# langtech-bsc/quantool

Measured on AMD Instinct MI355X. Metric: quantized weights/sec (GPTQ int4, Llama-3-8B, 512 calib samples), higher is better.
Workload: dtype f32

## Files before the change

### quantool_amd/csrc/cholesky.hip

```cpp
#include <stdlib.h>
#include <string.h>

#include <map>
#include <tuple>
#include <vector>

#include "common.h"
#include "gemm3_tn.h"
#include "sgemm_tn.h"

namespace {

constexpr int NB = 128;
constexpr int NBO_MAX = 1024;
static int chol_block_env(const char* name) {
    const char* e = getenv(name);
    if (!e) return 0;
    int x = atoi(e) / 128 * 128;
    return x < 128 ? 128 : (x > NBO_MAX ? NBO_MAX : x);
}
struct G3Step {
    int n_items = 0, n_red = 0;
    size_t item_off = 0, red_off = 0;
};
// ... 316 lines not shown
#pragma unroll
        for (int a = 0; a < 4; ++a)
#pragma unroll
            for (int r = 0; r < 16; ++r) {
                const int row = 32 * a + (r & 3) + 8 * (r >> 2) + 4 * h;
                if (row < n) Z[(size_t)row * ldz + col] = acc[a][r];
            }
    }
}

__global__ __launch_bounds__(128) void trinv_batched_kernel(const float* __restrict__ Rd_all, int K,
                                                            float* __restrict__ Dinv_all,
                                                            float* __restrict__ Y, int64_t ldy, int64_t bsW, int64_t bsY) {
    if (blockIdx.y) {
        Rd_all += (size_t)blockIdx.y * bsW;
        Dinv_all += (size_t)blockIdx.y * bsW;
        Y += (size_t)blockIdx.y * bsY;
    }
    extern __shared__ __attribute__((aligned(16))) float sm[];
    float* Rt = sm;
    float* Xs = sm + NB * LDT;
    const int b = blockIdx.x;
    const int n = (K - b * NB < NB) ? K - b * NB : NB;
    const float* Rd = Rd_all + (size_t)b * RD_STRIDE;
    const int j = threadIdx.x;
    for (int e = j; e < NB * NB; e += NB) {
        const int i = e / NB, c = e % NB;
        Rt[c * LDT + i] = Rd[e];
    }
    __syncthreads();
    float x0[32], x1[32], x2[32], x3[32];
#pragma unroll
    for (int r = 0; r < 32; ++r) {
        x0[r] = (r == j) ? 1.0f : 0.0f;
        x1[r] = (32 + r == j) ? 1.0f : 0.0f;
        x2[r] = (64 + r == j) ? 1.0f : 0.0f;
        x3[r] = (96 + r == j) ? 1.0f : 0.0f;
    }
#pragma unroll 1
    for (int pb = 3; pb >= 0; --pb) {
#pragma unroll
        for (int pp = 31; pp >= 0; --pp) {
            const int p = 32 * pb + pp;
            const float* rp = Rt + p * LDT;
            const float xp = QT_SEL4(pb, x0[pp], x1[pp], x2[pp], x3[pp]) / rp[p];
            if (pb == 0) x0[pp] = xp;
            if (pb == 1) x1[pp] = xp;
            if (pb == 2) x2[pp] = xp;
            if (pb == 3) x3[pp] = xp;
#define QT_XUPD(arr, a, r_to)                                                 \
    _Pragma("unroll") for (int r4 = 0; r4 < (r_to); r4 += 4) {                 \
        const f32x4 v4 = *(const f32x4*)(rp + 32 * (a) + r4);                 \
        _Pragma("unroll") for (int e = 0; e < 4; ++e)                         \
            if (r4 + e < (r_to)) arr[r4 + e] = fmaf(-v4[e], xp, arr[r4 + e]); \
    }
            if (pb == 0) { QT_XUPD(x0, 0, pp) } else { QT_XUPD(x0, 0, 32) }
            if (pb == 1) { QT_XUPD(x1, 1, pp) } else if (pb > 1) { QT_XUPD(x1, 1, 32) }
            if (pb == 2) { QT_XUPD(x2, 2, pp) } else if (pb > 2) { QT_XUPD(x2, 2, 32) }
            if (pb == 3) { QT_XUPD(x3, 3, pp) }
#undef QT_XUPD
        }
    }
#pragma unroll
    for (int r = 0; r < 32; ++r) {
        Xs[r * LDP + j] = x0[r];
        Xs[(32 + r) * LDP + j] = x1[r];
        Xs[(64 + r) * LDP + j] = x2[r];
        Xs[(96 + r) * LDP + j] = x3[r];
    }
    __syncthreads();
    float* Dinv = Dinv_all + (size_t)b * NB * NB;
    float* Yd = Y + (size_t)(b * NB) * ldy + b * NB;
    for (int e = j; e < NB * NB; e += NB) {
        const int i = e / NB, jj = e % NB;
        const bool in = (i < n && jj < n);
        Dinv[e] = (in && jj >= i) ? Xs[i * LDP + jj] : 0.0f;
        if (in) Yd[(size_t)i * ldy + jj] = (jj <= i) ? Xs[jj * LDP + i] : 0.0f;
    }
}

__global__ __launch_bounds__(256) void trinv_mfma_kernel(const float* __restrict__ Rd_all, int K,
                                                         float* __restrict__ Dinv_all,
                                                         float* __restrict__ Y, int64_t ldy, int64_t bsW, int64_t bsY) {
    if (blockIdx.y) {
        Rd_all += (size_t)blockIdx.y * bsW;
        Dinv_all += (size_t)blockIdx.y * bsW;
        Y += (size_t)blockIdx.y * bsY;
    }
    extern __shared__ __attribute__((aligned(16))) float Rs[];
    const int blk = blockIdx.x;
    const int n = (K - blk * NB < NB) ? K - blk * NB : NB;
    const float* Rd = Rd_all + (size_t)blk * RD_STRIDE;
    const int tid = threadIdx.x, lane = tid & 63, wave = tid >> 6;
    {
        constexpr int NV = RD_STRIDE / 4 / 256;
        f32x4 v[NV];
#pragma unroll
        for (int r = 0; r < NV; ++r) v[r] = ((const f32x4*)Rd)[tid + 256 * r];
#pragma unroll
        for (int r = 0; r < NV; ++r) ((f32x4*)Rs)[tid + 256 * r] = v[r];
    }
    const float* D32 = Rs + NB * NB;
    const int l31 = lane & 31, h = lane >> 5;
    const int col = wave * 32 + l31;

    f32x16 acc[4];
#pragma unroll
    for (int a = 0; a < 4; ++a)
#pragma unroll
        for (int r = 0; r < 16; ++r) {
            const int row = 32 * a + (r & 3) + 8 * (r >> 2) + 4 * h;
            acc[a][r] = (row == col) ? 1.0f : 0.0f;
        }
    __syncthreads();

#pragma unroll
    for (int b = 0; b < 4; ++b) {
        f32x16 zb;
#pragma unroll
        for (int r = 0; r < 16; ++r) zb[r] = 0.0f;
#pragma unroll
        for (int r = 0; r < 16; ++r) {
            const int k = (r & 3) + 8 * (r >> 2) + 4 * h;
            const float av = D32[(b * 32 + k) * 32 + l31];
            zb = __builtin_amdgcn_mfma_f32_32x32x2f32(av, acc[b][r], zb, 0, 0, 0);
        }
        acc[b] = zb;
#pragma unroll
        for (int a = b + 1; a < 4; ++a) {
#pragma unroll
            for (int r = 0; r < 16; ++r) {
                const int k = (r & 3) + 8 * (r >> 2) + 4 * h;
                const float av = -Rs[(32 * b + k) * NB + 32 * a + l31];
                acc[a] = __builtin_amdgcn_mfma_f32_32x32x2f32(av, zb[r], acc[a], 0, 0, 0);
            }
        }
    }
    float* Dinv = Dinv_all + (size_t)blk * NB * NB;
    float* Yd = Y + (size_t)(blk * NB) * ldy + blk * NB;
#pragma unroll
    for (int a = 0; a < 4; ++a)
#pragma unroll
        for (int r = 0; r < 16; ++r) {
            const int row = 32 * a + (r & 3) + 8 * (r >> 2) + 4 * h;
            const bool in = row < n && col < n;
            const float z = (in && row >= col) ? acc[a][r] : 0.0f;
            Dinv[col * NB + row] = z;
            if (in) Yd[(size_t)row * ldy + col] = z;
        }
}

__global__ __launch_bounds__(256) void transpose_lower_block_kernel(const float* __restrict__ Y, int64_t ldy, int w,
                                                                    float* __restrict__ XT, int ldx, int64_t bsY,
                                                                    int64_t bsXT) {
    if (blockIdx.z) {
        Y += (size_t)blockIdx.z * bsY;
        XT += (size_t)blockIdx.z * bsXT;
    }
    __shared__ float tile[32][33];
    const int bx = blockIdx.x * 32, by = blockIdx.y * 32;
    const int tx = threadIdx.x & 31, ty = threadIdx.x >> 5;
    for (int r = ty; r < 32; r += 8) {
        const int m = bx + r, k = by + tx;
        tile[r][tx] = (m < w && k < w && k <= m) ? Y[(size_t)m * ldy + k] : 0.0f;
    }
    __syncthreads();
    for (int r = ty; r < 32; r += 8) {
        const int k = by + r, m = bx + tx;
        if (k < w && m < w) XT[(size_t)k * ldx + m] = tile[tx][r];
    }
}

__global__ __launch_bounds__(256) void flat_reverse_lower_to_upper_kernel(float* __restrict__ U, int K, int64_t bsU) {
    U += (size_t)blockIdx.z * bsU;
    const int j = blockIdx.x * blockDim.x + threadIdx.x;
    const int i = blockIdx.y;
    if (j >= K || j < i) return;
    const size_t e = (size_t)i * K + j;
    const size_t pe = (size_t)(K - 1 - i) * K + (K - 1 - j);
    if (i == j) {
        if (e <= pe) {
            const float t = U[e];
            U[e] = U[pe];
            U[pe] = t;
        }
    } else {
        U[e] = U[pe];
        U[pe] = 0.0f;
    }
}

__global__ __launch_bounds__(256) void identity_if_failed_kernel(float* __restrict__ U, int K,
                                                                 const int32_t* __restrict__ info, int64_t bsU) {
    if (info[blockIdx.z] == 0) return;
    U += (size_t)blockIdx.z * bsU;
    for (int i = blockIdx.x; i < K; i += gridDim.x)
        for (int j = threadIdx.x; j < K; j += blockDim.x) U[(size_t)i * K + j] = (i == j) ? 1.0f : 0.0f;
}

}

static size_t chol_problem_ws_bytes(int K, const CholG3Plan* g3) {
    const size_t nb = (K + NB - 1) / NB;
    const size_t split = (size_t)2048 * NB * NB * 4 + (size_t)NBO_MAX * K * 4;
    size_t n = (size_t)NB * K * 4 + (size_t)NBO_MAX * K * 4 + (size_t)NBO_MAX * NBO_MAX * 4 + nb * (NB * NB + RD_STRIDE) * 4 + split + 256;
    if (g3->any) n += 2 * qt_align_up((size_t)3 * K * K * 2, 256) + (size_t)g3->max_slabs * 256 * 256 * 4 + 256;
    return qt_align_up(n, 256);
}

extern "C" size_t qt_cholesky_inverse_upper_batched_workspace_bytes(int K, int n_problems) {
    if (K <= 0 || n_problems <= 0) return 0;
    int nbo_, nbi_;
    const CholG3Plan* g3 = chol_blocks(K, nbo_, nbi_);
    return (size_t)n_problems * chol_problem_ws_bytes(K, g3) + g3->blob_bytes + 512;
}

extern "C" size_t qt_cholesky_inverse_upper_workspace_bytes(int K) {
    return qt_cholesky_inverse_upper_batched_workspace_bytes(K, 1);
}

static int chol_run(float* A, int64_t strideA, int K, float* U, int64_t strideU, int32_t* info, int nprob, void* workspace,
                    size_t workspace_bytes, hipStream_t stream) {
    const size_t need = qt_cholesky_inverse_upper_batched_workspace_bytes(K, nprob);
    if (!workspace || workspace_bytes < need) {
        qt_set_error("qt_cholesky_inverse_upper: workspace %zu < required %zu", workspace_bytes, need);
        return QT_ERR_WORKSPACE;
    }
    const int nblk = (K + NB - 1) / NB;
    char* ws = (char*)qt_align_up((size_t)workspace, 256);
    int NBO, NBI;
    const CholG3Plan* g3 = chol_blocks(K, NBO, NBI);
    const size_t prob_bytes = chol_problem_ws_bytes(K, g3);
    const int64_t sW = (int64_t)(prob_bytes / 4);
    const int64_t sA = nprob > 1 ? strideA : 0, sU = nprob > 1 ? strideU : 0;
    float* T = (float*)ws;
    float* TI = T + (size_t)NB * K;
    float* XT = TI + (size_t)NBO_MAX * K;
    float* Rd = XT + (size_t)NBO_MAX * NBO_MAX;
    float* Dinv = Rd + (size_t)nblk * RD_STRIDE;
    float* split_ws = Dinv + (size_t)nblk * NB * NB;
    const size_t split_ws_bytes = (size_t)2048 * NB * NB * 4 + (size_t)NBO_MAX * K * 4;
    unsigned short *Rpl = nullptr, *Ypl = nullptr;
    float* g3_slabs = nullptr;
    char* g3_tab = nullptr;
    const int64_t plane_stride = (int64_t)K * K;
    if (g3->any) {
        char* q = (char*)qt_align_up((size_t)((char*)split_ws + split_ws_bytes), 256);
        Rpl = (unsigned short*)q;
        q += qt_align_up((size_t)3 * K * K * 2, 256);
        Ypl = (unsigned short*)q;
        q += qt_align_up((size_t)3 * K * K * 2, 256);
        g3_slabs = (float*)q;
        g3_tab = (char*)qt_align_up((size_t)(ws + (size_t)nprob * prob_bytes), 256);
        QT_HIP(hipMemcpyAsync(g3_tab, g3->blob, g3->blob_bytes, hipMemcpyHostToDevice, stream));
    }
    auto g3_row = [&](const G3Step& st, const unsigned short* Bplanes, int col_a0, int col_b0, int M, int N, float* C,
                      int64_t bsC, int mode) -> int {
        G3Args a;
        a.Apl = Rpl;
        a.Bpl = Bplanes;
        a.plane_stride = plane_stride;
        a.ld = K;
        a.rowA0 = a.rowB0 = 0;
        a.colA0 = col_a0;
        a.colB0 = col_b0;
        a.colmax = K;
        a.M = M;
        a.N = N;
        a.C = C;
        a.ldc = K;
        a.mode = mode;
        a.slabs = g3_slabs;
        a.items = (const G3Item*)(g3_tab + st.item_off);
        a.n_items = st.n_items;
        a.red = (const G3Red*)(g3_tab + st.red_off);
        a.n_red = st.n_red;
        a.batch = nprob;
        a.bsApl = a.bsBpl = sW * 2;
        a.bsC = bsC;
        a.bsSlabs = sW;
        return qt_gemm3_launch(a, stream);
    };
    auto sgemm = [&](SgemmArgs& g, int64_t bsA_, int64_t bsB_, int64_t bsC_) -> int {
        g.batch = nprob;
        g.bsA = bsA_;
        g.bsB = bsB_;
        g.bsCin = g.bsCout = bsC_;
        g.bs_split = sW;
        return qt_sgemm_tn(g, stream);
    };
    float* Y = U;
    const int64_t sY = sU;
    const size_t inv_lds = (size_t)(NB * LDT + NB * LDP) * sizeof(float);
    const size_t potf2_lds = (size_t)(NB * LDA + 4 * 32 * 32) * sizeof(float);
    static QtOncePerDevice lds_attr;
    QT_HIP(lds_attr.run([&] {
        hipError_t e = hipFuncSetAttribute((const void*)potf2_kernel, hipFuncAttributeMaxDynamicSharedMemorySize,
                                           (int)potf2_lds);
        if (e == hipSuccess)
            e = hipFuncSetAttribute((const void*)trsm_rt_kernel, hipFuncAttributeMaxDynamicSharedMemorySize,
                                    (int)(RD_STRIDE * sizeof(float)));
        if (e == hipSuccess)
            e = hipFuncSetAttribute((const void*)trinv_batched_kernel, hipFuncAttributeMaxDynamicSharedMemorySize,
                                    (int)inv_lds);
        if (e == hipSuccess)
            e = hipFuncSetAttribute((const void*)trinv_mfma_kernel, hipFuncAttributeMaxDynamicSharedMemorySize,
                                    (int)(RD_STRIDE * sizeof(float)));
        return e;
    }));
    QT_HIP(hipMemsetAsync(info, 0, sizeof(int32_t) * nprob, stream));
    const int prio = qt_chain_prio();

    for (int J0 = 0, Jb = 0; J0 < K; J0 += NBO, ++Jb) {
        const int J1 = (K - J0 < NBO) ? K : J0 + NBO;
        if (g3->any && J0 > 0) {
            const G3Step& st = g3->fac[Jb];
            float* C = A + (size_t)J0 * K + J0;
            if (st.n_items > 0) {
                int rc = g3_row(st, Rpl, J0, J0, J1 - J0, K - J0, C, sA, G3_SUB);
                if (rc) return rc;
            } else {
                SgemmArgs g;
                g.A = A + J0; g.lda = K;
                g.B = A + J0; g.ldb = K;
                g.Cin = C; g.ldcin = K;
                g.Cout = C; g.ldcout = K;
                g.M = J1 - J0; g.N = K - J0; g.kdim = J0; g.k_mode = SG_K_FULL; g.mode = SG_MODE_SUB;
                g.split_ws = split_ws; g.split_ws_bytes = split_ws_bytes;
                int rc = sgemm(g, sA, sA, sA);
                if (rc) return rc;
            }
        }
        for (int j0 = J0; j0 < J1; j0 += NB) {
            const int j = j0 / NB, nbj = (K - j0 < NB) ? K - j0 : NB;
            float* Ajj = A + (size_t)j0 * K + j0;
            if (j0 > J0) {
                SgemmArgs g;
                g.A = A + (size_t)J0 * K + j0; g.lda = K;
                g.B = A + (size_t)J0 * K + j0; g.ldb = K;
                g.Cin = Ajj; g.ldcin = K;
                g.Cout = Ajj; g.ldcout = K;
                g.M = nbj; g.N = K - j0; g.kdim = j0 - J0; g.k_mode = SG_K_FULL; g.mode = SG_MODE_SUB;
                int rc = sgemm(g, sA, sA, sA);
                if (rc) return rc;
            }
            hipLaunchKernelGGL(potf2_kernel, dim3(nprob), dim3(POTF2_THREADS), potf2_lds, stream, (const float*)Ajj, (int64_t)K, nbj,
                               Ajj, (int64_t)K, Rd + (size_t)j * RD_STRIDE, info, j0, prio, sA, sW);
            QT_LAUNCH_CHECK();
            const int rest = K - j0 - nbj;
            if (rest > 0) {
                hipLaunchKernelGGL(trsm_rt_kernel, dim3((rest + 127) / 128, nprob), dim3(256), RD_STRIDE * sizeof(float),
                                   stream, (const float*)(Rd + (size_t)j * RD_STRIDE), nbj, (const float*)(Ajj + nbj),
                                   (int64_t)K, Ajj + nbj, (int64_t)K, rest, prio, sW, sA);
                QT_LAUNCH_CHECK();
            }
        }
        const int rem = K - J1;
        if (g3->any) {
            if (rem > 0) {
                int rc = qt_split3_launch(A + (size_t)J0 * K + J0, K, J1 - J0, K - J0, Rpl + (size_t)J0 * K + J0, K,
                                          plane_stride, 0, 0, 0, stream, nprob, sA, sW * 2);
                if (rc) return rc;
            }
        } else if (rem > 0) {
            SgemmArgs g;
            g.A = A + (size_t)J0 * K + J1; g.lda = K;
            g.B = A + (size_t)J0 * K + J1; g.ldb = K;
            g.Cin = A + (size_t)J1 * K + J1; g.ldcin = K;
            g.Cout = A + (size_t)J1 * K + J1; g.ldcout = K;
            g.M = rem; g.N = rem; g.kdim = J1 - J0; g.k_mode = SG_K_FULL; g.mode = SG_MODE_SUB;
            g.upper_only = 1;
            int rc = sgemm(g, sA, sA, sA);
            if (rc) return rc;
        }
    }
    {
        const char* e = getenv("QT_CHOL_TRINV");
        if (e && strcmp(e, "div") == 0)
            hipLaunchKernelGGL(trinv_batched_kernel, dim3(nblk, nprob), dim3(NB), inv_lds, stream, (const float*)Rd, K, Dinv, Y,
                               (int64_t)K, sW, sY);
        else
            hipLaunchKernelGGL(trinv_mfma_kernel, dim3(nblk, nprob), dim3(256), RD_STRIDE * sizeof(float), stream,
                               (const float*)Rd, K, Dinv, Y, (int64_t)K, sW, sY);
    }
    QT_LAUNCH_CHECK();
    for (int I0 = 0, Ib = 0; I0 < K; I0 += NBI, ++Ib) {
        const int I1 = (K - I0 < NBI) ? K : I0 + NBI;
        const int Wi = I1 - I0;
        for (int i0 = I0 + NB; i0 < I1; i0 += NB) {
            const int i = i0 / NB, nbi = (K - i0 < NB) ? K - i0 : NB;
            SgemmArgs g;
            g.A = A + (size_t)I0 * K + i0; g.lda = K;
            g.B = Y + (size_t)I0 * K + I0; g.ldb = K;
            g.Cin = nullptr; g.ldcin = 0;
            g.Cout = T; g.ldcout = K;
            g.M = nbi; g.N = i0 - I0; g.kdim = i0 - I0; g.k_mode = SG_K_FROM_N0; g.mode = SG_MODE_SET;
            int rc = sgemm(g, sA, sY, sW);
            if (rc) return rc;
            SgemmArgs t;
            t.A = Dinv + (size_t)i * NB * NB; t.lda = NB;
            t.B = T; t.ldb = K;
            t.Cin = nullptr; t.ldcin = 0;
            t.Cout = Y + (size_t)i0 * K + I0; t.ldcout = K;
            t.M = nbi; t.N = i0 - I0; t.kdim = nbi; t.k_mode = SG_K_FULL; t.mode = SG_MODE_NEG;
            rc = sgemm(t, sW, sW, sY);
            if (rc) return rc;
        }
        auto split_row = [&]() -> int {
            if (!g3->any || I1 >= K) return QT_OK;
            return qt_split3_launch(Y + (size_t)I0 * K, K, Wi, I1, Ypl + (size_t)I0 * K, K, plane_stride, 1, I0, 0, stream,
                                    nprob, sY, sW * 2);
        };
        if (I0 == 0) {
            int rc0 = split_row();
            if (rc0) return rc0;
            continue;
        }
        int rc;
        if (g3->any && g3->inv[Ib].n_items > 0) {
            rc = g3_row(g3->inv[Ib], Ypl, I0, 0, Wi, I0, TI, sW, G3_SET);
        } else {
            SgemmArgs g;
            g.A = A + I0; g.lda = K;
            g.B = Y; g.ldb = K;
            g.Cin = nullptr; g.ldcin = 0;
            g.Cout = TI; g.ldcout = K;
            g.M = Wi; g.N = I0; g.kdim = I0; g.k_mode = SG_K_FROM_N0; g.mode = SG_MODE_SET;
            g.split_ws = split_ws; g.split_ws_bytes = split_ws_bytes;
            rc = sgemm(g, sA, sY, sW);
        }
        if (rc) return rc;
        hipLaunchKernelGGL(transpose_lower_block_kernel, dim3((Wi + 31) / 32, (Wi + 31) / 32, nprob), dim3(256), 0, stream,
                           (const float*)(Y + (size_t)I0 * K + I0), (int64_t)K, Wi, XT, NBO_MAX, sY, sW);
        QT_LAUNCH_CHECK();
        SgemmArgs t;
        t.A = XT; t.lda = NBO_MAX;
        t.B = TI; t.ldb = K;
        t.Cin = nullptr; t.ldcin = 0;
        t.Cout = Y + (size_t)I0 * K; t.ldcout = K;
        t.M = Wi; t.N = I0; t.kdim = Wi; t.k_mode = SG_K_FULL; t.mode = SG_MODE_NEG;
        rc = sgemm(t, sW, sW, sY);
        if (rc) return rc;
        rc = split_row();
        if (rc) return rc;
    }
    hipLaunchKernelGGL(flat_reverse_lower_to_upper_kernel, dim3((K + 255) / 256, K, nprob), dim3(256), 0, stream, U, K, sU);
    QT_LAUNCH_CHECK();
    hipLaunchKernelGGL(identity_if_failed_kernel, dim3(K < 1024 ? K : 1024, 1, nprob), dim3(256), 0, stream, U, K,
                       (const int32_t*)info, sU);
    QT_LAUNCH_CHECK();
    return QT_OK;
}

extern "C" int qt_cholesky_inverse_upper(float* A, int K, float* U, int32_t* info, void* workspace,
                                         size_t workspace_bytes, qt_stream_t stream_) {
    QT_CHECK_ARG(K > 0 && A && U && info, "qt_cholesky_inverse_upper: bad arguments");
    return chol_run(A, 0, K, U, 0, info, 1, workspace, workspace_bytes, (hipStream_t)stream_);
}

extern "C" int qt_cholesky_inverse_upper_batched(float* A, int64_t strideA, int K, float* U, int64_t strideU, int32_t* info,
                                                 int n_problems, void* workspace, size_t workspace_bytes,
                                                 qt_stream_t stream_) {
    QT_CHECK_ARG(K > 0 && A && U && info && n_problems >= 1 && n_problems <= SG_MAX_BATCH,
                 "qt_cholesky_inverse_upper_batched: bad arguments (1 <= n_problems <= %d)", SG_MAX_BATCH);
    QT_CHECK_ARG(n_problems == 1 || (strideA >= (int64_t)K * K && strideU >= (int64_t)K * K && strideA % 4 == 0 && strideU % 4 == 0),
                 "qt_cholesky_inverse_upper_batched: strides must be multiples of 4 elements and >= K*K");
    return chol_run(A, strideA, K, U, strideU, info, n_problems, workspace, workspace_bytes, (hipStream_t)stream_);
}
```

### quantool_amd/csrc/sgemm_tn.h

```cpp
#pragma once
#include "common.h"

enum { SG_MODE_SUB = 0, SG_MODE_SET = 1, SG_MODE_NEG = 2 };
enum { SG_K_FULL = 0, SG_K_FROM_N0 = 1 };
constexpr int SG_MAX_GROUPS = 16;
constexpr int SG_MAX_BATCH = 16;

struct SgemmArgs {
    const float* A; int64_t lda;
    const float* B; int64_t ldb;
    const float* Cin; int64_t ldcin;
    float* Cout; int64_t ldcout;
    int M, N, kdim;
    int k_mode;
    int mode;
    float* split_ws = nullptr;
    size_t split_ws_bytes = 0;
    int chain_len = 0;
    int upper_only = 0;
    int batch = 1;
    int64_t bsA = 0, bsB = 0, bsCin = 0, bsCout = 0;
    int64_t bs_split = 0;
    int n_groups = 0;
    int64_t group_bsB = 0;
    int group_m_end[SG_MAX_GROUPS] = {};
    int k_chunk = 0;
    int n_splits = 1;
    int fast_interior = 1;
};

int qt_sgemm_tn(const SgemmArgs& a, hipStream_t stream);

int qt_splitk_reduce(const float* slabs, int splits, int M, int N, const float* Cin, int64_t ldcin, float* Cout,
                     int64_t ldcout, int mode, hipStream_t stream, int batch = 1, int64_t bs_slabs = 0, int64_t bs_cin = 0,
                     int64_t bs_cout = 0);
```

### quantool_amd/csrc/sgemm_tn.hip

```cpp
#include <stdlib.h>

#include <type_traits>

#include "ring_pipe.h"
#include "sgemm_tn.h"

namespace {

constexpr int BK = 16;

#ifndef QT_SGEMM_PD
#define QT_SGEMM_PD 2
#endif

template <int N, class F>
__device__ __forceinline__ void sg_static_for(F&& f) {
    if constexpr (N > 0) {
        sg_static_for<N - 1>(f);
        f(std::integral_constant<int, N - 1>{});
    }
}

template <int BM, int BN, int MODE, bool CHAIN = false, int NWAVE = 4>
__global__ __launch_bounds__(64 * NWAVE) __attribute__((amdgpu_waves_per_eu(NWAVE == 8 ? 4 : 2))) void sgemm_tn_kernel(const SgemmArgs p) {
    constexpr int NT = 64 * NWAVE;
    constexpr int WGM = NWAVE == 8 ? 4 : 2, WGN = 2;
    constexpr int WM = BM / (32 * WGM), WN = BN / (32 * WGN);
    constexpr int A4 = BK * BM / 4 / NT;
    constexpr int B4 = BK * BN / 4 / NT;
    static_assert(A4 >= 1 && B4 >= 1, "tile too small for the workgroup");
    __shared__ __attribute__((aligned(16))) float As[2][BK][BM];
    __shared__ __attribute__((aligned(16))) float Bs[2][BK][BN];

    const int tid = threadIdx.x, lane = tid & 63, wave = tid >> 6;
    const int wave_m = wave >> 1, wave_n = wave & 1;
    const int m0 = blockIdx.y * BM, n0 = blockIdx.x * BN;
    if (p.upper_only && m0 >= n0 + BN) return;
    const float* Ap = p.A;
    const float* Bp = p.B;
    const float* Cinp = p.Cin;
    float* Coutp = p.Cout;
    int zsplit = blockIdx.z;
    if (p.batch > 1) {
        const int b = zsplit / p.n_splits;
        zsplit -= b * p.n_splits;
        Ap += (size_t)b * p.bsA;
        Bp += (size_t)b * p.bsB;
        if (Cinp) Cinp += (size_t)b * p.bsCin;
        Coutp += (size_t)b * p.bsCout;
    }
    if (p.n_groups > 0) {
        int g = 0;
        while (g + 1 < p.n_groups && m0 >= p.group_m_end[g]) ++g;
        Bp += (size_t)g * p.group_bsB;
    }
    const bool tile_inside = p.fast_interior && m0 + BM <= p.M && n0 + BN <= p.N;

    int k_begin = 0;
    if (p.k_mode == SG_K_FROM_N0) k_begin = n0 / BK * BK;
    int k_end = p.kdim;
    if (p.k_chunk > 0) {
        const int lo = zsplit * p.k_chunk, hi = lo + p.k_chunk;
        k_begin = k_begin > lo ? k_begin : lo;
        k_end = k_end < hi ? k_end : hi;
        Coutp += (size_t)zsplit * (size_t)p.M * (size_t)p.N;
    }

    const bool a_vec = (p.lda % 4 == 0) && (((uintptr_t)Ap & 15) == 0);
    const bool b_vec = (p.ldb % 4 == 0) && (((uintptr_t)Bp & 15) == 0);

    constexpr int PD = (BM == 64 && BN == 64 && !CHAIN) ? QT_SGEMM_PD : 1;
    static_assert(PD == 1 || PD % 2 == 0, "the LDS buffer of a step is s & 1: the unrolled ring must be even");
    f32x4 ra[PD][A4], rb[PD][B4];

    const bool interior = p.fast_interior && a_vec && b_vec && m0 + BM <= p.M && n0 + BN <= p.N;
    auto gload_fast = [&](int k0, auto slot_c) {
        constexpr int slot = decltype(slot_c)::value;
#pragma unroll
        for (int r = 0; r < A4; ++r) {
            const int idx = tid + NT * r;
            ra[slot][r] = *(const f32x4*)(Ap + (size_t)(k0 + idx / (BM / 4)) * p.lda + m0 + (idx % (BM / 4)) * 4);
        }
#pragma unroll
        for (int r = 0; r < B4; ++r) {
            const int idx = tid + NT * r;
            rb[slot][r] = *(const f32x4*)(Bp + (size_t)(k0 + idx / (BN / 4)) * p.ldb + n0 + (idx % (BN / 4)) * 4);
        }
    };
    auto gload = [&](int k0, auto slot_c) {
        constexpr int slot = decltype(slot_c)::value;
        if (interior && k0 + BK <= k_end) {
            gload_fast(k0, slot_c);
            return;
        }
#pragma unroll
        for (int r = 0; r < A4; ++r) {
            const int idx = tid + NT * r;
            const int kr = idx / (BM / 4), c = (idx % (BM / 4)) * 4;
            const int k = k0 + kr, m = m0 + c;
            f32x4 v = {0.f, 0.f, 0.f, 0.f};
            if (k < k_end) {
                const float* src = Ap + (size_t)k * p.lda + m;
                if (a_vec && m + 3 < p.M) {
                    v = *(const f32x4*)src;
                } else {
#pragma unroll
                    for (int e = 0; e < 4; ++e)
                        if (m + e < p.M) v[e] = src[e];
                }
            }
            ra[slot][r] = v;
        }
#pragma unroll
        for (int r = 0; r < B4; ++r) {
            const int idx = tid + NT * r;
            const int kr = idx / (BN / 4), c = (idx % (BN / 4)) * 4;
            const int k = k0 + kr, n = n0 + c;
            f32x4 v = {0.f, 0.f, 0.f, 0.f};
            if (k < k_end) {
                const float* src = Bp + (size_t)k * p.ldb + n;
                if (b_vec && n + 3 < p.N) {
                    v = *(const f32x4*)src;
                } else {
#pragma unroll
                    for (int e = 0; e < 4; ++e)
                        if (n + e < p.N) v[e] = src[e];
                }
            }
            rb[slot][r] = v;
        }
    };
    auto lstore = [&](int buf, auto slot_c) {
        constexpr int slot = decltype(slot_c)::value;
#pragma unroll
        for (int r = 0; r < A4; ++r) {
            const int idx = tid + NT * r;
            *(f32x4*)&As[buf][idx / (BM / 4)][(idx % (BM / 4)) * 4] = ra[slot][r];
        }
#pragma unroll
        for (int r = 0; r < B4; ++r) {
            const int idx = tid + NT * r;
            *(f32x4*)&Bs[buf][idx / (BN / 4)][(idx % (BN / 4)) * 4] = rb[slot][r];
        }
    };

    f32x16 acc[WM][WN];
#pragma unroll
    for (int i = 0; i < WM; ++i)
#pragma unroll
        for (int j = 0; j < WN; ++j)
#pragma unroll
            for (int r = 0; r < 16; ++r) acc[i][j][r] = 0.0f;

    const int h = lane >> 5, l31 = lane & 31;
    f32x16 cpre[WM][WN];
    if (MODE == SG_MODE_SUB) {
#pragma unroll
        for (int i = 0; i < WM; ++i)
#pragma unroll
            for (int j = 0; j < WN; ++j)
#pragma unroll
                for (int r = 0; r < 16; ++r) {
                    const int row = m0 + wave_m * (BM / WGM) + i * 32 + (r & 3) + 8 * (r >> 2) + 4 * h;
                    const int col = n0 + wave_n * (BN / WGN) + j * 32 + l31;
                    cpre[i][j][r] = (tile_inside || (row < p.M && col < p.N)) ? Cinp[(size_t)row * p.ldcin + col] : 0.0f;
                }
    }
    const int nsteps = (k_end - k_begin + BK - 1) / BK;
    auto kstep = [&](int s, auto u_c, auto fast_c) {
        constexpr int u = decltype(u_c)::value;
        constexpr bool FAST = decltype(fast_c)::value;
        const int buf = s & 1;
        if constexpr (FAST) {
            const int sn = s + PD < nsteps ? s + PD : nsteps - 1;
            gload_fast(k_begin + sn * BK, std::integral_constant<int, u>{});
        } else {
            if (s + PD < nsteps) gload(k_begin + (s + PD) * BK, std::integral_constant<int, u>{});
        }
#pragma unroll
        for (int kk = 0; kk < BK / 2; ++kk) {
                float a[WM], b[WN];
#pragma unroll
                for (int i = 0; i < WM; ++i) a[i] = As[buf][2 * kk + h][wave_m * (BM / WGM) + i * 32 + l31];
#pragma unroll
                for (int j = 0; j < WN; ++j) b[j] = Bs[buf][2 * kk + h][wave_n * (BN / WGN) + j * 32 + l31];
#pragma unroll
                for (int i = 0; i < WM; ++i)
#pragma unroll
                    for (int j = 0; j < WN; ++j)
                        acc[i][j] = __builtin_amdgcn_mfma_f32_32x32x2f32(a[i], b[j], acc[i][j], 0, 0, 0);
            }
        if (FAST || s + 1 < nsteps) lstore(buf ^ 1, std::integral_constant<int, (u + 1) % PD>{});
        if (CHAIN && s + 1 < nsteps && ((s + 1) * BK) % p.chain_len == 0) {
#pragma unroll
            for (int i = 0; i < WM; ++i)
#pragma unroll
// ... 133 lines not shown
                int m0i, n0i;
                size_t oa, ob, oci, oco;
                tile_origin(is_it, m0i, n0i, oa, ob, oci, oco);
                is_a = p.A + oa + m0i;
                is_b = p.B + ob + n0i;
            }
        } else {
            is_a += a_step;
            is_b += b_step;
        }
    };
    static_assert((RS & (RS - 1)) == 0, "slot = stream index & (RS - 1)");

    f32x16 acc[2], cpre[2];
    const int cvoff_in = (int)(((size_t)(4 * h) * (size_t)p.ldcin + (size_t)l31) * 4);
    const int cvoff_out = (int)(((size_t)(4 * h) * (size_t)p.ldcout + (size_t)l31) * 4);
    const int cstep_in = (int)((size_t)p.ldcin * 4), cstep_out = (int)((size_t)p.ldcout * 4);
    size_t c_off_in = 0, c_off_out = 0;
    auto load_c = [&](int m0, int n0) {
        const int rw = m0 + wave_m * 32, cw = n0 + wave_n * 64;
        const auto rs = __builtin_amdgcn_make_buffer_rsrc((void*)(p.Cin + c_off_in + (size_t)rw * p.ldcin + cw), 0, 0x7FFFFFFF, 0x00020000);
#pragma unroll
        for (int r = 0; r < 16; ++r) {
            const int soff = ((r & 3) + 8 * (r >> 2)) * cstep_in;
#pragma unroll
            for (int j = 0; j < 2; ++j)
                cpre[j][r] = __builtin_bit_cast(float, __builtin_amdgcn_raw_buffer_load_b32(rs, cvoff_in + j * 128, soff, 0));
        }
    };
    auto store_c = [&](int m0, int n0) {
        const int rw = m0 + wave_m * 32, cw = n0 + wave_n * 64;
        const auto rs = __builtin_amdgcn_make_buffer_rsrc((void*)(p.Cout + c_off_out + (size_t)rw * p.ldcout + cw), 0, 0x7FFFFFFF, 0x00020000);
#pragma unroll
        for (int r = 0; r < 16; ++r) {
            const int soff = ((r & 3) + 8 * (r >> 2)) * cstep_out;
#pragma unroll
            for (int j = 0; j < 2; ++j)
                __builtin_amdgcn_raw_buffer_store_b32(__builtin_bit_cast(unsigned, cpre[j][r] - acc[j][r]), rs, cvoff_out + j * 128, soff, 0);
        }
    };
    auto zero_acc = [&]() {
#pragma unroll
        for (int j = 0; j < 2; ++j)
#pragma unroll
            for (int r = 0; r < 16; ++r) acc[j][r] = 0.0f;
    };

    int m0, n0;
    {
        size_t oa, ob;
        tile_origin(0, m0, n0, oa, ob, c_off_in, c_off_out);
    }
    load_c(m0, n0);
    issue_next();
    issue_next();

    const int nchains = steps / fold_every;
    const int pairs_per_chain = fold_every / 2;
    int batch_prev = 0;
    int g = 0;
    for (int it = 0; it < my_tiles; ++it) {
        for (int ch = 0; ch < nchains; ++ch) {
            zero_acc();
            for (int ps = 0; ps < pairs_per_chain; ++ps, g += 2) {
                if (batch_prev) wait_vmcnt<32>();
                else wait_vmcnt<0>();
                __builtin_amdgcn_s_barrier();
                if (g + 2 < total) {
                    issue_next();
                    issue_next();
                }
                batch_prev = 0;
#pragma unroll
                for (int half = 0; half < 2; ++half) {
                    const char* stage = ring + ((g + half) & (RS - 1)) * RSTAGE_BYTES;
                    const float* As = (const float*)stage + wave_m * 32 + l31;
                    const float* Bs = (const float*)(stage + RBK * RBM * 4) + wave_n * 64 + l31;
#pragma unroll
                    for (int kk = 0; kk < RBK / 2; ++kk) {
                        const float a = As[(2 * kk + h) * RBM];
                        const float b0 = Bs[(2 * kk + h) * RBN], b1 = Bs[(2 * kk + h) * RBN + 32];
                        acc[0] = __builtin_amdgcn_mfma_f32_32x32x2f32(a, b0, acc[0], 0, 0, 0);
                        acc[1] = __builtin_amdgcn_mfma_f32_32x32x2f32(a, b1, acc[1], 0, 0, 0);
                    }
                }
                if (ps == 0 && ch == 0 && it > 0) {
                    load_c(m0, n0);
                    __builtin_amdgcn_sched_barrier(0);
                    batch_prev = 32;
                }
            }
            if (ch + 1 < nchains) {
#pragma unroll
                for (int j = 0; j < 2; ++j)
#pragma unroll
                    for (int r = 0; r < 16; ++r) cpre[j][r] = cpre[j][r] - acc[j][r];
            }
        }
        store_c(m0, n0);
        __builtin_amdgcn_sched_barrier(0);
        batch_prev = 32;
        if (it + 1 < my_tiles) {
            size_t oa, ob;
            tile_origin(it + 1, m0, n0, oa, ob, c_off_in, c_off_out);
        }
    }
}

__global__ __launch_bounds__(256) void splitk_reduce_kernel(const float* __restrict__ slabs, int splits, int M,
                                                            int N, const float* __restrict__ Cin, int64_t ldcin,
                                                            float* __restrict__ Cout, int64_t ldcout, int mode,
                                                            int64_t bs_slabs, int64_t bs_cin, int64_t bs_cout) {
    const int col = (blockIdx.x * blockDim.x + threadIdx.x) * 4;
    const int row = blockIdx.y;
    if (col >= N) return;
    if (blockIdx.z) {
        slabs += (size_t)blockIdx.z * bs_slabs;
        if (Cin) Cin += (size_t)blockIdx.z * bs_cin;
        Cout += (size_t)blockIdx.z * bs_cout;
    }
    const size_t mn = (size_t)M * N;
    if (col + 3 < N && (N & 3) == 0) {
        f32x4 s = {0.f, 0.f, 0.f, 0.f};
        const float* src = slabs + (size_t)row * N + col;
        int z = 0;
        for (; z + 8 <= splits; z += 8) {
            f32x4 v[8];
#pragma unroll
            for (int u = 0; u < 8; ++u) v[u] = *(const f32x4*)(src + (size_t)(z + u) * mn);
#pragma unroll
            for (int u = 0; u < 8; ++u) s += v[u];
        }
        for (; z < splits; ++z) s += *(const f32x4*)(src + (size_t)z * mn);
#pragma unroll
        for (int e = 0; e < 4; ++e) {
            float v = s[e];
            if (mode == SG_MODE_SUB) v = Cin[(size_t)row * ldcin + col + e] - v;
            if (mode == SG_MODE_NEG) v = -v;
            Cout[(size_t)row * ldcout + col + e] = v;
        }
    } else {
        for (int e = 0; e < 4 && col + e < N; ++e) {
            float v = 0.f;
            for (int z = 0; z < splits; ++z) v += slabs[z * mn + (size_t)row * N + col + e];
            if (mode == SG_MODE_SUB) v = Cin[(size_t)row * ldcin + col + e] - v;
            if (mode == SG_MODE_NEG) v = -v;
            Cout[(size_t)row * ldcout + col + e] = v;
        }
    }
}

template <int BM, int BN>
int launch(const SgemmArgs& a, hipStream_t stream, int splits = 1) {
    dim3 grid((a.N + BN - 1) / BN, (a.M + BM - 1) / BM, splits * (a.batch > 1 ? a.batch : 1));
    static const bool sub8 = [] {
        const char* e = getenv("QT_SGEMM_SUB_WAVES");
        return !(e && atoi(e) == 4);
    }();
    switch (a.mode) {
        case SG_MODE_SUB:
            if constexpr (BM == 128 && BN == 128) {
                if (sub8) {
                    if (a.chain_len > 0)
                        hipLaunchKernelGGL((sgemm_tn_kernel<BM, BN, SG_MODE_SUB, true, 8>), grid, dim3(512), 0, stream, a);
                    else
                        hipLaunchKernelGGL((sgemm_tn_kernel<BM, BN, SG_MODE_SUB, false, 8>), grid, dim3(512), 0, stream, a);
                    break;
                }
            }
            if (a.chain_len > 0)
                hipLaunchKernelGGL((sgemm_tn_kernel<BM, BN, SG_MODE_SUB, true>), grid, dim3(256), 0, stream, a);
            else
                hipLaunchKernelGGL((sgemm_tn_kernel<BM, BN, SG_MODE_SUB>), grid, dim3(256), 0, stream, a);
            break;
        case SG_MODE_SET:
            hipLaunchKernelGGL((sgemm_tn_kernel<BM, BN, SG_MODE_SET>), grid, dim3(256), 0, stream, a);
            break;
        default:
            hipLaunchKernelGGL((sgemm_tn_kernel<BM, BN, SG_MODE_NEG>), grid, dim3(256), 0, stream, a);
            break;
    }
    QT_LAUNCH_CHECK();
    return QT_OK;
}

}

int qt_splitk_reduce(const float* slabs, int splits, int M, int N, const float* Cin, int64_t ldcin, float* Cout,
                     int64_t ldcout, int mode, hipStream_t stream, int batch, int64_t bs_slabs, int64_t bs_cin,
                     int64_t bs_cout) {
    hipLaunchKernelGGL(splitk_reduce_kernel, dim3((N / 4 + 255) / 256 + 1, M, batch > 1 ? batch : 1), dim3(256), 0, stream,
                       slabs, splits, M, N, Cin, ldcin, Cout, ldcout, mode, bs_slabs, bs_cin, bs_cout);
    QT_LAUNCH_CHECK();
    return QT_OK;
}

int qt_sgemm_tn(const SgemmArgs& a_, hipStream_t stream) {
    if (a_.M <= 0 || a_.N <= 0) return QT_OK;
    QT_CHECK_ARG(a_.batch >= 1 && a_.batch <= SG_MAX_BATCH && a_.n_groups >= 0 && a_.n_groups <= SG_MAX_GROUPS &&
                     !(a_.batch > 1 && a_.n_groups > 0),
                 "qt_sgemm_tn: batch %d / row groups %d unsupported", a_.batch, a_.n_groups);
    for (int g = 0; g < a_.n_groups; ++g)
        QT_CHECK_ARG((a_.group_m_end[g] % 128 == 0 || g == a_.n_groups - 1) && (g == 0 || a_.group_m_end[g] >= a_.group_m_end[g - 1]),
                     "qt_sgemm_tn: row group %d ends at %d (boundaries must be ascending multiples of 128)", g, a_.group_m_end[g]);
    static const int fast_interior = [] {
        const char* e = getenv("QT_SGEMM_INTERIOR");
        return (e && atoi(e) == 0) ? 0 : 1;
    }();
    SgemmArgs a = a_;
    a.fast_interior = fast_interior;
    const long t128 = (long)((a.M + 127) / 128) * ((a.N + 127) / 128);
    if (a.split_ws && t128 < 384 && a.kdim >= 512) {
        static const int target_wgs = [] {
            const char* e = getenv("QT_SGEMM_SPLIT_TARGET");
            const int v = e ? atoi(e) : 256;
            return v < 256 ? 256 : v;
        }();
        static const int min_chunk = [] {
            const char* e = getenv("QT_SGEMM_SPLIT_MIN_CHUNK");
            const int v = e ? atoi(e) : 128;
            return v < 64 ? 64 : v;
        }();
        int splits = (int)(target_wgs / t128);
        if (splits > 32) splits = 32;
        if (splits < 1) splits = 1;
        int chunk = (a.kdim + splits - 1) / splits;
        chunk = (chunk + 63) / 64 * 64;
        if (chunk < min_chunk) chunk = min_chunk;
        splits = (a.kdim + chunk - 1) / chunk;
        const size_t need = (size_t)splits * a.M * a.N * sizeof(float);
        if (splits >= 2 && need <= a.split_ws_bytes && (a.batch <= 1 || (size_t)a.bs_split * sizeof(float) >= need)) {
            SgemmArgs part = a;
            part.Cin = nullptr;
            part.ldcin = 0;
            part.Cout = a.split_ws;
            part.ldcout = a.N;
            part.bsCin = 0;
            part.bsCout = a.bs_split;
            part.mode = SG_MODE_SET;
            part.k_chunk = chunk;
            part.n_splits = splits;
            const int rc = launch<128, 128>(part, stream, splits);
            if (rc) return rc;
            return qt_splitk_reduce(a.split_ws, splits, a.M, a.N, a.Cin, a.ldcin, a.Cout, a.ldcout, a.mode, stream, a.batch,
                                    a.bs_split, a.bsCin, a.bsCout);
        }
    }
    const char* ring_env = getenv("QT_SGEMM_RING");
    const int use_ring = (ring_env && atoi(ring_env) == 0) ? 0 : 1;
    const char* ring_min_env = getenv("QT_SGEMM_RING_MIN_TILES");
    const int ring_min_tiles = ring_min_env ? atoi(ring_min_env) : 32;
    if (use_ring && a.mode == SG_MODE_SUB && a.k_mode == SG_K_FULL && a.k_chunk == 0 && a.kdim >= 4 * RBK &&
        a.kdim % (2 * RBK) == 0 && (a.chain_len == 0 || (a.chain_len % (2 * RBK) == 0 && a.kdim % a.chain_len == 0)) &&
        a.kdim % RBK == 0 && (a.chain_len == 0 || a.chain_len % RBK == 0) && a.M % RBM == 0 && a.N % RBN == 0 &&
        (size_t)40 * (size_t)(a.ldcin > a.ldcout ? a.ldcin : a.ldcout) * 4 < ((size_t)1 << 31) && a.lda % 4 == 0 &&
        a.ldb % 4 == 0 && (((uintptr_t)a.A | (uintptr_t)a.B) & 15) == 0 &&
        (size_t)RBK * (size_t)(a.lda > a.ldb ? a.lda : a.ldb) * 4 < ((size_t)1 << 32) && (!a.upper_only || a.M == a.N)) {
        RingArgs r;
        r.A = a.A; r.lda = a.lda; r.B = a.B; r.ldb = a.ldb;
        r.Cin = a.Cin; r.ldcin = a.ldcin; r.Cout = a.Cout; r.ldcout = a.ldcout;
        r.M = a.M; r.N = a.N; r.kdim = a.kdim;
        r.chain_len = a.chain_len > 0 ? a.chain_len : a.kdim;
        const int tm = (a.M + RBM - 1) / RBM, tn = (a.N + RBN - 1) / RBN;
        r.tiles_n = tn;
        r.upper_only = a.upper_only;
        r.n_tiles = a.upper_only ? tn * (tn + 1) / 2 : tm * tn;
        r.batch = a.batch > 1 ? a.batch : 1;
        r.bsA = a.bsA; r.bsB = a.bsB; r.bsCin = a.bsCin; r.bsCout = a.bsCout;
        r.n_groups = a.n_groups;
        r.group_bsB = a.group_bsB;
        for (int g = 0; g < SG_MAX_GROUPS; ++g) r.group_m_end[g] = a.group_m_end[g];
        if (r.n_tiles >= ring_min_tiles) {
            const int all = r.n_tiles * r.batch;
            const int grid = all >= 2 * 256 ? 2 * 256 : all;
            hipLaunchKernelGGL(sgemm_ring_kernel, dim3(grid), dim3(512), 0, stream, r);
            QT_LAUNCH_CHECK();
            return QT_OK;
        }
    }
    if (t128 >= 384) return launch<128, 128>(a, stream);
    return launch<64, 64>(a, stream);
}

extern "C" size_t qt_sgemm_tn_f32_workspace_bytes(int M, int N) {
    if (M <= 0 || N <= 0) return 0;
    return (size_t)32 * M * N * 4 + 256;
}

extern "C" int qt_sgemm_tn_f32(const float* A, int64_t lda, const float* B, int64_t ldb, const float* Cin,
                               int64_t ldcin, float* Cout, int64_t ldcout, int M, int N, int kdim, int skip_zero_k,
                               int mode, int allow_split_k, void* workspace, size_t workspace_bytes,
                               qt_stream_t stream_) {
    hipStream_t stream = (hipStream_t)stream_;
    QT_CHECK_ARG(A && B && Cout && M > 0 && N > 0 && kdim >= 0, "qt_sgemm_tn_f32: bad arguments");
    QT_CHECK_ARG(mode == SG_MODE_SUB || mode == SG_MODE_SET || mode == SG_MODE_NEG, "qt_sgemm_tn_f32: mode %d", mode);
    QT_CHECK_ARG(mode != SG_MODE_SUB || Cin, "qt_sgemm_tn_f32: MODE_SUB needs Cin");
    SgemmArgs g;
    g.A = A; g.lda = lda;
    g.B = B; g.ldb = ldb;
    g.Cin = Cin; g.ldcin = ldcin;
    g.Cout = Cout; g.ldcout = ldcout;
    g.M = M; g.N = N; g.kdim = kdim;
    g.k_mode = skip_zero_k ? SG_K_FROM_N0 : SG_K_FULL;
    g.mode = mode;
    if (allow_split_k) {
        const size_t need = qt_sgemm_tn_f32_workspace_bytes(M, N);
        if (!workspace || workspace_bytes < need) {
            qt_set_error("qt_sgemm_tn_f32: workspace %zu < required %zu", workspace_bytes, need);
            return QT_ERR_WORKSPACE;
        }
        g.split_ws = (float*)qt_align_up((size_t)workspace, 256);
        g.split_ws_bytes = workspace_bytes - 256;
    }
    return qt_sgemm_tn(g, stream);
}
```

Before: 2.992 billion.

## Hoist diagonal-block triangular inverse steps across all block rows into batched launches

Adds a 'rows' batching dimension to the sgemm kernel and the transpose kernel, then runs the per-diagonal-block inner-inverse GEMM steps and transposes for all NBI block rows in one launch instead of once per outer row iteration. The aim is fewer small kernel launches and more workgroups per launch in the Cholesky-based inverse used by GPTQ. The cost is extra workspace for per-row XT buffers when they do not fit inside TI, a new argument check, and an env switch to turn it off. If the grid z dimension is large or the workspace aliasing is wrong, results could be corrupted.

```diff
diff --git a/quantool_amd/csrc/cholesky.hip b/quantool_amd/csrc/cholesky.hip
--- a/quantool_amd/csrc/cholesky.hip
+++ b/quantool_amd/csrc/cholesky.hip
@@ -492,10 +492,11 @@
 
 __global__ __launch_bounds__(256) void transpose_lower_block_kernel(const float* __restrict__ Y, int64_t ldy, int w,
                                                                     float* __restrict__ XT, int ldx, int64_t bsY,
-                                                                    int64_t bsXT) {
+                                                                    int64_t bsXT, int nprob, int64_t rsY, int64_t rsXT) {
     if (blockIdx.z) {
-        Y += (size_t)blockIdx.z * bsY;
-        XT += (size_t)blockIdx.z * bsXT;
+        const int r = blockIdx.z / nprob, b = blockIdx.z - r * nprob;
+        Y += (size_t)r * rsY + (size_t)b * bsY;
+        XT += (size_t)r * rsXT + (size_t)b * bsXT;
     }
     __shared__ float tile[32][33];
     const int bx = blockIdx.x * 32, by = blockIdx.y * 32;
@@ -540,11 +541,16 @@
 
 }
 
-static size_t chol_problem_ws_bytes(int K, const CholG3Plan* g3) {
+static size_t chol_xt_rows_extra_bytes(int K, int NBI) {
+    return 2 * NBI <= NBO_MAX ? 0 : (size_t)NBI * K * 4;
+}
+
+static size_t chol_problem_ws_bytes(int K, int NBI, const CholG3Plan* g3) {
     const size_t nb = (K + NB - 1) / NB;
     const size_t split = (size_t)2048 * NB * NB * 4 + (size_t)NBO_MAX * K * 4;
     size_t n = (size_t)NB * K * 4 + (size_t)NBO_MAX * K * 4 + (size_t)NBO_MAX * NBO_MAX * 4 + nb * (NB * NB + RD_STRIDE) * 4 + split + 256;
     if (g3->any) n += 2 * qt_align_up((size_t)3 * K * K * 2, 256) + (size_t)g3->max_slabs * 256 * 256 * 4 + 256;
+    n += chol_xt_rows_extra_bytes(K, NBI);
     return qt_align_up(n, 256);
 }
 
@@ -552,7 +558,7 @@
     if (K <= 0 || n_problems <= 0) return 0;
     int nbo_, nbi_;
     const CholG3Plan* g3 = chol_blocks(K, nbo_, nbi_);
-    return (size_t)n_problems * chol_problem_ws_bytes(K, g3) + g3->blob_bytes + 512;
+    return (size_t)n_problems * chol_problem_ws_bytes(K, nbi_, g3) + g3->blob_bytes + 512;
 }
 
 extern "C" size_t qt_cholesky_inverse_upper_workspace_bytes(int K) {
@@ -570,7 +576,7 @@
     char* ws = (char*)qt_align_up((size_t)workspace, 256);
     int NBO, NBI;
     const CholG3Plan* g3 = chol_blocks(K, NBO, NBI);
-    const size_t prob_bytes = chol_problem_ws_bytes(K, g3);
+    const size_t prob_bytes = chol_problem_ws_bytes(K, NBI, g3);
     const int64_t sW = (int64_t)(prob_bytes / 4);
     const int64_t sA = nprob > 1 ? strideA : 0, sU = nprob > 1 ? strideU : 0;
     float* T = (float*)ws;
@@ -584,6 +590,8 @@
     float* g3_slabs = nullptr;
     char* g3_tab = nullptr;
     const int64_t plane_stride = (int64_t)K * K;
+    const bool xt_in_ti = chol_xt_rows_extra_bytes(K, NBI) == 0;
+    float* XTall = xt_in_ti ? TI + (size_t)NBI * K : (float*)((char*)split_ws + split_ws_bytes);
     if (g3->any) {
         char* q = (char*)qt_align_up((size_t)((char*)split_ws + split_ws_bytes), 256);
         Rpl = (unsigned short*)q;
@@ -591,6 +599,7 @@
         Ypl = (unsigned short*)q;
         q += qt_align_up((size_t)3 * K * K * 2, 256);
         g3_slabs = (float*)q;
+        if (!xt_in_ti) XTall = g3_slabs + (size_t)g3->max_slabs * 256 * 256;
         g3_tab = (char*)qt_align_up((size_t)(ws + (size_t)nprob * prob_bytes), 256);
         QT_HIP(hipMemcpyAsync(g3_tab, g3->blob, g3->blob_bytes, hipMemcpyHostToDevice, stream));
     }
@@ -724,26 +733,62 @@
                                (const float*)Rd, K, Dinv, Y, (int64_t)K, sW, sY);
     }
     QT_LAUNCH_CHECK();
-    for (int I0 = 0, Ib = 0; I0 < K; I0 += NBI, ++Ib) {
-        const int I1 = (K - I0 < NBI) ? K : I0 + NBI;
-        const int Wi = I1 - I0;
-        for (int i0 = I0 + NB; i0 < I1; i0 += NB) {
+    const char* hoist_env = getenv("QT_CHOL_DIAG_HOIST");
+    const bool hoist = !(hoist_env && atoi(hoist_env) == 0) && NBI > NB && K > NB;
+    const int64_t row_step = (int64_t)NBI * (K + 1);
+    auto diag_steps = [&](int I0, int W, int rows, float* Tslot) -> int {
+        for (int i0 = I0 + NB; i0 < I0 + W; i0 += NB) {
             const int i = i0 / NB, nbi = (K - i0 < NB) ? K - i0 : NB;
             SgemmArgs g;
             g.A = A + (size_t)I0 * K + i0; g.lda = K;
             g.B = Y + (size_t)I0 * K + I0; g.ldb = K;
             g.Cin = nullptr; g.ldcin = 0;
-            g.Cout = T; g.ldcout = K;
+            g.Cout = Tslot; g.ldcout = K;
             g.M = nbi; g.N = i0 - I0; g.kdim = i0 - I0; g.k_mode = SG_K_FROM_N0; g.mode = SG_MODE_SET;
+            g.rows = rows; g.rsA = row_step; g.rsB = row_step; g.rsCout = NBI;
             int rc = sgemm(g, sA, sY, sW);
             if (rc) return rc;
             SgemmArgs t;
             t.A = Dinv + (size_t)i * NB * NB; t.lda = NB;
-            t.B = T; t.ldb = K;
+            t.B = Tslot; t.ldb = K;
             t.Cin = nullptr; t.ldcin = 0;
             t.Cout = Y + (size_t)i0 * K + I0; t.ldcout = K;
             t.M = nbi; t.N = i0 - I0; t.kdim = nbi; t.k_mode = SG_K_FULL; t.mode = SG_MODE_NEG;
+            t.rows = rows; t.rsA = (int64_t)(NBI / NB) * NB * NB; t.rsB = NBI; t.rsCout = row_step;
             rc = sgemm(t, sW, sW, sY);
+            if (rc) return rc;
+        }
+        return QT_OK;
+    };
+    auto transpose_rows = [&](int I0, int W, int rows, float* XTdst, int ldx) {
+        hipLaunchKernelGGL(transpose_lower_block_kernel, dim3((W + 31) / 32, (W + 31) / 32, rows * nprob), dim3(256), 0, stream,
+                           (const float*)(Y + (size_t)I0 * K + I0), (int64_t)K, W, XTdst, ldx, sY, sW, nprob, row_step,
+                           (int64_t)NBI * NBI);
+    };
+    if (hoist) {
+        const int full_rows = K / NBI, tail0 = full_rows * NBI;
+        if (full_rows > 0) {
+            int rc = diag_steps(0, NBI, full_rows, T);
+            if (rc) return rc;
+        }
+        if (tail0 < K) {
+            int rc = diag_steps(tail0, K - tail0, 1, T + tail0);
+            if (rc) return rc;
+        }
+        if (full_rows > 1) {
+            transpose_rows(NBI, NBI, full_rows - 1, XTall + (size_t)NBI * NBI, NBI);
+            QT_LAUNCH_CHECK();
+        }
+        if (tail0 < K && tail0 > 0) {
+            transpose_rows(tail0, K - tail0, 1, XTall + (size_t)full_rows * NBI * NBI, NBI);
+            QT_LAUNCH_CHECK();
+        }
+    }
+    for (int I0 = 0, Ib = 0; I0 < K; I0 += NBI, ++Ib) {
+        const int I1 = (K - I0 < NBI) ? K : I0 + NBI;
+        const int Wi = I1 - I0;
+        if (!hoist) {
+            int rc = diag_steps(I0, Wi, 1, T);
             if (rc) return rc;
         }
         auto split_row = [&]() -> int {
@@ -770,11 +815,12 @@
             rc = sgemm(g, sA, sY, sW);
         }
         if (rc) return rc;
-        hipLaunchKernelGGL(transpose_lower_block_kernel, dim3((Wi + 31) / 32, (Wi + 31) / 32, nprob), dim3(256), 0, stream,
-                           (const float*)(Y + (size_t)I0 * K + I0), (int64_t)K, Wi, XT, NBO_MAX, sY, sW);
-        QT_LAUNCH_CHECK();
+        if (!hoist) {
+            transpose_rows(I0, Wi, 1, XT, NBO_MAX);
+            QT_LAUNCH_CHECK();
+        }
         SgemmArgs t;
-        t.A = XT; t.lda = NBO_MAX;
+        t.A = hoist ? XTall + (size_t)Ib * NBI * NBI : XT; t.lda = hoist ? NBI : NBO_MAX;
         t.B = TI; t.ldb = K;
         t.Cin = nullptr; t.ldcin = 0;
         t.Cout = Y + (size_t)I0 * K; t.ldcout = K;
diff --git a/quantool_amd/csrc/sgemm_tn.h b/quantool_amd/csrc/sgemm_tn.h
--- a/quantool_amd/csrc/sgemm_tn.h
+++ b/quantool_amd/csrc/sgemm_tn.h
@@ -21,6 +21,8 @@
     int batch = 1;
     int64_t bsA = 0, bsB = 0, bsCin = 0, bsCout = 0;
     int64_t bs_split = 0;
+    int rows = 1;
+    int64_t rsA = 0, rsB = 0, rsCin = 0, rsCout = 0;
     int n_groups = 0;
     int64_t group_bsB = 0;
     int group_m_end[SG_MAX_GROUPS] = {};
diff --git a/quantool_amd/csrc/sgemm_tn.hip b/quantool_amd/csrc/sgemm_tn.hip
--- a/quantool_amd/csrc/sgemm_tn.hip
+++ b/quantool_amd/csrc/sgemm_tn.hip
@@ -41,7 +41,15 @@
     const float* Cinp = p.Cin;
     float* Coutp = p.Cout;
     int zsplit = blockIdx.z;
-    if (p.batch > 1) {
+    if (p.rows > 1) {
+        const int nb = p.batch > 1 ? p.batch : 1;
+        const int r = zsplit / nb, b = zsplit - r * nb;
+        zsplit = 0;
+        Ap += (size_t)r * p.rsA + (size_t)b * p.bsA;
+        Bp += (size_t)r * p.rsB + (size_t)b * p.bsB;
+        if (Cinp) Cinp += (size_t)r * p.rsCin + (size_t)b * p.bsCin;
+        Coutp += (size_t)r * p.rsCout + (size_t)b * p.bsCout;
+    } else if (p.batch > 1) {
         const int b = zsplit / p.n_splits;
         zsplit -= b * p.n_splits;
         Ap += (size_t)b * p.bsA;
@@ -481,7 +489,7 @@
 
 template <int BM, int BN>
 int launch(const SgemmArgs& a, hipStream_t stream, int splits = 1) {
-    dim3 grid((a.N + BN - 1) / BN, (a.M + BM - 1) / BM, splits * (a.batch > 1 ? a.batch : 1));
+    dim3 grid((a.N + BN - 1) / BN, (a.M + BM - 1) / BM, splits * (a.batch > 1 ? a.batch : 1) * (a.rows > 1 ? a.rows : 1));
     static const bool sub8 = [] {
         const char* e = getenv("QT_SGEMM_SUB_WAVES");
         return !(e && atoi(e) == 4);
@@ -529,6 +537,9 @@
     QT_CHECK_ARG(a_.batch >= 1 && a_.batch <= SG_MAX_BATCH && a_.n_groups >= 0 && a_.n_groups <= SG_MAX_GROUPS &&
                      !(a_.batch > 1 && a_.n_groups > 0),
                  "qt_sgemm_tn: batch %d / row groups %d unsupported", a_.batch, a_.n_groups);
+    QT_CHECK_ARG(a_.rows >= 1 && (a_.rows == 1 || (a_.split_ws == nullptr && a_.n_groups == 0 && a_.mode != SG_MODE_SUB &&
+                                                   a_.chain_len == 0 && (long)a_.rows * a_.batch <= 65535)),
+                 "qt_sgemm_tn: rows %d need MODE_SET / MODE_NEG without split-K, row groups or chains", a_.rows);
     for (int g = 0; g < a_.n_groups; ++g)
         QT_CHECK_ARG((a_.group_m_end[g] % 128 == 0 || g == a_.n_groups - 1) && (g == 0 || a_.group_m_end[g] >= a_.group_m_end[g - 1]),
                      "qt_sgemm_tn: row group %d ends at %d (boundaries must be ascending multiples of 128)", g, a_.group_m_end[g]);
```

Result: no change. 3.010 billion (median of 6 runs) (+0.6%).
